# PJLab-ADG/DetZero

Measured on AMD Instinct MI355X. Metric: LiDAR frames/sec (160k pts, 0.1m voxels), higher is better.
Workload: dtype f32 as f16 pairs (hi+lo, 22-bit significand; 3 f16 MFMA per product, f32 accumulate)

## Files before the change

### detzero_amd/csrc/head_cand.hip

```cpp
#include "hgemm.h"

namespace dz {

constexpr int HC_C = 64;
constexpr int HC_CAND = 32;
constexpr int HC_THREADS = 192;
constexpr int HC_PIX_BYTES = HC_C * 4;
constexpr int HC_HROW = HC_PIX_BYTES + 16;
constexpr int HC_LDS_BYTES = 9 * HC_CAND * HC_HROW;
constexpr int HC_MAX_BRANCH = 4;

struct HcArgs {
    const unsigned char *shared;
    const unsigned long long *cand;
    const int *ncand;
    const unsigned char *w1, *w2;
    const float *s1, *b1, *s2, *b2;
    float *head;
    int h, w, k, cand_stride, w1_cout;
    int g_cout[HC_MAX_BRANCH], g_ooff[HC_MAX_BRANCH];
};

template <class M>
__global__ __launch_bounds__(HC_THREADS) __attribute__((amdgpu_waves_per_eu(2, 2))) void k_head_at_cand(HcArgs a) {
    extern __shared__ __attribute__((aligned(16))) unsigned char hid_s[];
    const int tid = threadIdx.x, lane = tid & 63, ty = tid >> 6;
    const int n = lane & 31, hh = lane >> 5;
    const int g = blockIdx.y, b = blockIdx.z;
    const int hw = a.h * a.w, hp = a.h + 2, wp = a.w + 2;
    const int ncand = min(min(a.ncand[b], a.k), a.cand_stride);
    const int slot = blockIdx.x * HC_CAND + n;
    if (blockIdx.x * HC_CAND >= ncand) return;
    const bool live = slot < ncand;
    int pix = 0, y = 0, x = 0;
    if (live) {
        const unsigned long long e = a.cand[(size_t)b * a.cand_stride + slot];
        const uint32_t flat = 0xFFFFFFFFu - (uint32_t)(e & 0xFFFFFFFFull);
        pix = (int)(flat % (uint32_t)hw);
        y = pix / a.w;
        x = pix - y * a.w;
    }
    const int hy = y + ty - 1;
    bool ok[3];
    const unsigned char *base[3];
#pragma unroll
    for (int tx = 0; tx < 3; ++tx) {
        const int hx = x + tx - 1;
        ok[tx] = live && hy >= 0 && hy < a.h && hx >= 0 && hx < a.w;
        base[tx] = a.shared + (ok[tx] ? (((size_t)b * hp + hy) * wp + hx) * HC_PIX_BYTES : (size_t)0);
    }
    f32x16 acc[2][3];
#pragma unroll
    for (int ct = 0; ct < 2; ++ct)
#pragma unroll
        for (int tx = 0; tx < 3; ++tx)
#pragma unroll
            for (int e = 0; e < 16; ++e) acc[ct][tx][e] = 0.f;
    const v4u zero4 = {0u, 0u, 0u, 0u};
    const unsigned char *const wrow = a.w1 + ((size_t)(g * HC_C + n) * HC_C) * 4;
    const size_t w_tap = (size_t)a.w1_cout * HC_C * 4, w_ct = (size_t)32 * HC_C * 4;
    for (int kc = 0; kc < HC_C / 32; ++kc) {
#pragma unroll
        for (int s = 0; s < 9; ++s) {
            const int ky = s / 3, kx = s - ky * 3;
            const size_t toff = (size_t)(ky * wp + kx) * HC_PIX_BYTES;
#pragma unroll
            for (int q = 0; q < 2; ++q) {
                const int koff = kc * 128 + q * 64 + hh * 32;
                v4u c_hi[2], c_lo[2], p_hi[3], p_lo[3];
#pragma unroll
                for (int ct = 0; ct < 2; ++ct) {
                    const unsigned char *wpn = wrow + s * w_tap + ct * w_ct + koff;
                    c_hi[ct] = *reinterpret_cast<const v4u *>(wpn);
                    c_lo[ct] = *reinterpret_cast<const v4u *>(wpn + 16);
                }
#pragma unroll
                for (int tx = 0; tx < 3; ++tx) {
                    p_hi[tx] = p_lo[tx] = zero4;
                    if (ok[tx]) {
                        const unsigned char *pp = base[tx] + toff + koff;
                        p_hi[tx] = *reinterpret_cast<const v4u *>(pp);
                        p_lo[tx] = *reinterpret_cast<const v4u *>(pp + 16);
                    }
                }
#pragma unroll
                for (int term = 3 - M::TERMS; term < 3; ++term)
#pragma unroll
                    for (int ct = 0; ct < 2; ++ct)
#pragma unroll
                        for (int tx = 0; tx < 3; ++tx)
                            acc[ct][tx] = M::mma(term == 0 ? c_lo[ct] : c_hi[ct], term == 1 ? p_lo[tx] : p_hi[tx], acc[ct][tx]);
            }
        }
    }
#pragma unroll
    for (int tx = 0; tx < 3; ++tx) {
        unsigned char *const row = hid_s + ((ty * 3 + tx) * HC_CAND + n) * HC_HROW;
#pragma unroll
        for (int ct = 0; ct < 2; ++ct) {
#pragma unroll
            for (int j = 0; j < 4; ++j) {
                const int ch = g * HC_C + ct * 32 + 8 * j + 4 * hh;
                float v[4];
#pragma unroll
                for (int e = 0; e < 4; ++e) v[e] = fmaxf(fmaf(acc[ct][tx][4 * j + e], a.s1[ch + e], a.b1[ch + e]), 0.f);
                uint2 hi, lo;
                split4<M>(v, hi, lo);
                if (!ok[tx]) hi = lo = make_uint2(0u, 0u);
                unsigned char *d = row + (ct * 4 + j) * 32 + hh * 8;
                *reinterpret_cast<uint2 *>(d) = hi;
                *reinterpret_cast<uint2 *>(d + 16) = lo;
            }
        }
    }
    __syncthreads();
    if (ty != 0) return;
    f32x16 out;
#pragma unroll
    for (int e = 0; e < 16; ++e) out[e] = 0.f;
    const unsigned char *const w2row = a.w2 + ((size_t)(g * 9 * 32 + n) * HC_C) * 4;
    for (int kc = 0; kc < HC_C / 32; ++kc) {
#pragma unroll
        for (int s = 0; s < 9; ++s) {
#pragma unroll
            for (int q = 0; q < 2; ++q) {
                const int koff = kc * 128 + q * 64 + hh * 32;
                const unsigned char *wpn = w2row + (size_t)s * 32 * HC_C * 4 + koff;
                const v4u c_hi = *reinterpret_cast<const v4u *>(wpn), c_lo = *reinterpret_cast<const v4u *>(wpn + 16);
                const unsigned char *pp = hid_s + (s * HC_CAND + n) * HC_HROW + koff;
                const v4u p_hi = *reinterpret_cast<const v4u *>(pp), p_lo = *reinterpret_cast<const v4u *>(pp + 16);
                if constexpr (M::TERMS == 3) {
                    out = M::mma(c_lo, p_hi, out);
                    out = M::mma(c_hi, p_lo, out);
                }
                out = M::mma(c_hi, p_hi, out);
            }
        }
    }
    if (live && hh == 0) {
        float *o = a.head + ((size_t)b * hw + pix) * 12 + a.g_ooff[g];
        const int gc = a.g_cout[g];
#pragma unroll
        for (int e = 0; e < 4; ++e) {
            if (e < gc) o[e] = fmaf(out[e], a.s2 ? a.s2[g * 32 + e] : 1.f, a.b2 ? a.b2[g * 32 + e] : 0.f);
        }
    }
}


constexpr int HF_CAND = 16;
constexpr int HF_HROW = HC_C + 4;

__global__ __launch_bounds__(HC_THREADS) void k_head_at_cand_f32(HcArgs a) {
    __shared__ __attribute__((aligned(16))) float hid_s[9 * HF_CAND * HF_HROW];
    __shared__ int pix_s[HF_CAND];
    __shared__ int ok_s[3][HF_CAND];
    const int tid = threadIdx.x, lane = tid & 63, ty = tid >> 6;
    const int r = lane & 15, g4 = lane >> 4;
    const int br = blockIdx.y, b = blockIdx.z;
    const int hw = a.h * a.w, hp = a.h + 2, wp = a.w + 2;
    const int ncand = min(min(a.ncand[b], a.k), a.cand_stride);
    if (blockIdx.x * HF_CAND >= ncand) return;
    const int slot = blockIdx.x * HF_CAND + r;
    const bool live = slot < ncand;
    int pix = 0, y = 0, x = 0;
    if (live) {
        const unsigned long long e = a.cand[(size_t)b * a.cand_stride + slot];
        const uint32_t flat = 0xFFFFFFFFu - (uint32_t)(e & 0xFFFFFFFFull);
        pix = (int)(flat % (uint32_t)hw);
        y = pix / a.w;
        x = pix - y * a.w;
    }
    const int hy = y + ty - 1;
    bool ok[3];
    const float *base[3];
    int okm = 0;
#pragma unroll
    for (int tx = 0; tx < 3; ++tx) {
        const int hx = x + tx - 1;
        ok[tx] = live && hy >= 0 && hy < a.h && hx >= 0 && hx < a.w;
        okm |= ok[tx] ? 1 << tx : 0;
        base[tx] = reinterpret_cast<const float *>(a.shared) + (ok[tx] ? (((size_t)b * hp + hy) * wp + hx) * HC_C : (size_t)0);
    }
    if (lane < HF_CAND) {
        ok_s[ty][lane] = okm;
        if (ty == 0) pix_s[lane] = live ? pix : -1;
    }
    __syncthreads();
    f32x4 acc[3][4];
#pragma unroll
    for (int tx = 0; tx < 3; ++tx)
#pragma unroll
        for (int nt = 0; nt < 4; ++nt) acc[tx][nt] = f32x4{0.f, 0.f, 0.f, 0.f};
    const float *const w1 = reinterpret_cast<const float *>(a.w1) + br * HC_C + r;
    for (int s = 0; s < 9; ++s) {
        const int ky = s / 3, kx = s - ky * 3;
        const size_t toff = (size_t)(ky * wp + kx) * HC_C;
#pragma unroll
        for (int kq = 0; kq < HC_C / 16; ++kq) {
            const int k0 = kq * 16 + g4 * 4;
            f32x4 av[3];
#pragma unroll
            for (int tx = 0; tx < 3; ++tx) {
                av[tx] = f32x4{0.f, 0.f, 0.f, 0.f};
                if (ok[tx]) av[tx] = *reinterpret_cast<const f32x4 *>(base[tx] + toff + k0);
            }
#pragma unroll
            for (int e = 0; e < 4; ++e) {
                float bv[4];
#pragma unroll
                for (int nt = 0; nt < 4; ++nt) bv[nt] = w1[((size_t)s * HC_C + k0 + e) * a.w1_cout + nt * 16];
#pragma unroll
                for (int tx = 0; tx < 3; ++tx)
#pragma unroll
                    for (int nt = 0; nt < 4; ++nt) acc[tx][nt] = __builtin_amdgcn_mfma_f32_16x16x4f32(av[tx][e], bv[nt], acc[tx][nt], 0, 0, 0);
            }
        }
    }
#pragma unroll
    for (int nt = 0; nt < 4; ++nt) {
        const int ch = br * HC_C + nt * 16 + r;
        const float sc = a.s1[ch], sh = a.b1[ch];
#pragma unroll
        for (int tx = 0; tx < 3; ++tx)
#pragma unroll
            for (int e = 0; e < 4; ++e) {
                const int c = 4 * g4 + e;
                const float v = fmaxf(fmaf(acc[tx][nt][e], sc, sh), 0.f);
                hid_s[((ty * 3 + tx) * HF_CAND + c) * HF_HROW + nt * 16 + r] = ((ok_s[ty][c] >> tx) & 1) ? v : 0.f;
            }
    }
    __syncthreads();
    if (ty != 0) return;
    f32x4 out = {0.f, 0.f, 0.f, 0.f};
    const float *const w2 = reinterpret_cast<const float *>(a.w2) + (size_t)br * 9 * HC_C * 16 + r;
    for (int s = 0; s < 9; ++s) {
#pragma unroll
        for (int kq = 0; kq < HC_C / 16; ++kq) {
            const int k0 = kq * 16 + g4 * 4;
            const f32x4 av = *reinterpret_cast<const f32x4 *>(hid_s + (s * HF_CAND + r) * HF_HROW + k0);
#pragma unroll
            for (int e = 0; e < 4; ++e) out = __builtin_amdgcn_mfma_f32_16x16x4f32(av[e], w2[((size_t)s * HC_C + k0 + e) * 16], out, 0, 0, 0);
        }
    }
    if (r < a.g_cout[br]) {
        const float sc = a.s2 ? a.s2[br * 16 + r] : 1.f, sh = a.b2 ? a.b2[br * 16 + r] : 0.f;
#pragma unroll
        for (int e = 0; e < 4; ++e) {
            const int px = pix_s[4 * g4 + e];
            if (px >= 0) a.head[((size_t)b * hw + px) * 12 + a.g_ooff[br] + r] = fmaf(out[e], sc, sh);
        }
    }
}

template <class M>
static int launch_head_at_cand(const HcArgs &a, int batch, int nbranch, hipStream_t stream) {
    static PerDeviceFlags lds_done;
    if (int rc_ = reserve_lds(reinterpret_cast<const void *>(&k_head_at_cand<M>), HC_LDS_BYTES, lds_done, "dz_head_at_candidates")) return rc_;
    hipLaunchKernelGGL((k_head_at_cand<M>), dim3(ceil_div(a.k, HC_CAND), nbranch, batch), dim3(HC_THREADS), HC_LDS_BYTES, stream, a);
    DZ_LAUNCH_CHECK();
    return DZ_OK;
}

}

using namespace dz;

extern "C" {

int dz_head_at_candidates_supported(int math, int channels) {
    return (math == DZ_MATH_F32 || math == DZ_MATH_F16X2 || math == DZ_MATH_BF16X2 || math == DZ_MATH_F16) && channels == HC_C ? 1 : 0;
}

int dz_head_at_candidates(const float *shared, int batch, int h, int w, const unsigned long long *cand, const int *d_ncand, int cand_stride,
                          int k, const float *w1, int w1_cout, const float *s1, const float *b1, const float *w2, const float *s2,
                          const float *b2, int nbranch, const int *h_g_cout, const int *h_g_ooff, float *head, int math, void *stream_) {
    hipStream_t stream = (hipStream_t)stream_;
    DZ_CHECK_ARG(dz_head_at_candidates_supported(math, HC_C), "dz_head_at_candidates: unknown math mode %d", math);
    DZ_CHECK_ARG(batch >= 0 && batch <= 65535 && h >= 1 && w >= 1 && k >= 1 && cand_stride >= k, "dz_head_at_candidates: bad sizes");
    DZ_CHECK_ARG(nbranch >= 1 && nbranch <= HC_MAX_BRANCH && w1_cout >= nbranch * HC_C && w1_cout % 32 == 0, "dz_head_at_candidates: bad branch layout");
    DZ_CHECK_ARG(shared && cand && d_ncand && w1 && s1 && b1 && w2 && head && h_g_cout && h_g_ooff, "dz_head_at_candidates: null pointer");
    if (batch == 0) return DZ_OK;
    HcArgs a{};
    for (int g = 0; g < nbranch; ++g) {
        DZ_CHECK_ARG(h_g_cout[g] >= 1 && h_g_cout[g] <= 4 && h_g_ooff[g] >= 0 && h_g_ooff[g] + h_g_cout[g] <= 12, "dz_head_at_candidates: bad columns of branch %d", g);
        a.g_cout[g] = h_g_cout[g];
        a.g_ooff[g] = h_g_ooff[g];
    }
    a.shared = reinterpret_cast<const unsigned char *>(shared);
    a.cand = cand; a.ncand = d_ncand;
    a.w1 = reinterpret_cast<const unsigned char *>(w1); a.w2 = reinterpret_cast<const unsigned char *>(w2);
    a.s1 = s1; a.b1 = b1; a.s2 = s2; a.b2 = b2; a.head = head;
    a.h = h; a.w = w; a.k = k; a.cand_stride = cand_stride; a.w1_cout = w1_cout;
    if (math == DZ_MATH_F32) {
        hipLaunchKernelGGL(k_head_at_cand_f32, dim3(ceil_div(k, HF_CAND), nbranch, batch), dim3(HC_THREADS), 0, stream, a);
        DZ_LAUNCH_CHECK();
        return DZ_OK;
    }
    if (math == DZ_MATH_F16X2) return launch_head_at_cand<MathF16>(a, batch, nbranch, stream);
    if (math == DZ_MATH_F16) return launch_head_at_cand<MathF16H>(a, batch, nbranch, stream);
    return launch_head_at_cand<MathBF16>(a, batch, nbranch, stream);
}

}
```

### detzero_amd/det_modules.py

```python
import contextlib
import os
from functools import partial

import numpy as np
import torch
import torch.nn as nn

from . import ops
from .lib import DetZeroHipError

PACKED_TABLES = bool(os.environ.get('DZ_TUNE_PACKED_TABLES'))

K3, S1, P1 = (3, 3, 3), (1, 1, 1), (1, 1, 1)


def _inference_only(module):
    if module.training:
        raise DetZeroHipError('%s: only the inference path is implemented on the HIP backend '
                              '(call .eval()); training is out of scope' % type(module).__name__)


def fold_bn(bn, conv_bias=None):
    w = bn.weight.detach().double()
    b = bn.bias.detach().double()
# ... 430 lines not shown
            e_prev, e = e, self._e('x_conv%d' % (i + 2))
            x = ops.spconv_forward(x, nbr_d, nxt, *self._p(dp, e_prev, e), None, True, in_level=level, math=mm)
            for bp in p[name]['blocks']:
                x = self._res_block(x, nbr, nxt, bp, e)
            nxt.act_exp = e
            out['x_conv%d' % (i + 2)] = (x, nxt)
            level = nxt
        dp = p['conv_out']
        nbr_d, _, nxt, ev = steps[4]
        ready(ev)
        e_prev, e = e, self._e('encoded')
        x = ops.spconv_forward(x, nbr_d, nxt, *self._p(dp, e_prev, e), None, True, in_level=level, math=mm)
        nxt.act_exp = e
        out['encoded'] = (x, nxt)
        return out

    def run(self, voxel_features, voxel_coords, batch_size, d_n=None, side_key=0, exact=False):
        return self.run_pyramid(self.build_pyramid(voxel_features, voxel_coords, batch_size, d_n, True, side_key, exact=exact))

    def _side_stream(self, dev, key=0):
        pool = self.__dict__.setdefault('_side_streams', {})
        k = (str(dev), key)
        if k not in pool:
            pool[k] = torch.cuda.Stream(device=dev, priority=int(os.environ.get('DZ_TUNE_SIDE_PRIORITY', '0')))
        return pool[k]

    def forward(self, batch_dict):
        _inference_only(self)
        vf = batch_dict['voxel_features'].float().contiguous()
        vc = batch_dict['voxel_coords'].int().contiguous()
        batch_size = batch_dict['batch_size']
        with torch.no_grad():
            res = self.run(vf, vc, batch_size, exact=True)

        def as_tensor(item):
            feats, level = item
            m = level.num_active()
            return SparseConvTensor(None, level.coords[:m], level.shape, batch_size, level=level, padded=(feats, level), math=self.math)
        batch_dict.update({'encoded_spconv_tensor': as_tensor(res['encoded']), 'encoded_spconv_tensor_stride': 8})
        batch_dict.update({'multi_scale_3d_features': {k: as_tensor(res[k]) for k in ('x_conv1', 'x_conv2', 'x_conv3', 'x_conv4')}})
        batch_dict.update({'multi_scale_3d_strides': {'x_conv1': 1, 'x_conv2': 2, 'x_conv3': 4, 'x_conv4': 8}})
        return batch_dict


class HeightCompression(nn.Module):

    def __init__(self, model_cfg, **kwargs):
        super().__init__()
        self.model_cfg = model_cfg
        self.num_bev_features = self.model_cfg.NUM_BEV_FEATURES

    def forward(self, batch_dict):
        t = batch_dict['encoded_spconv_tensor']
        feats, level = t._padded if t._padded is not None else (t.features, t._level)
        math = t._math if t._padded is not None else 0
        c = feats.shape[1]
        bev = ops.sparse_to_bev(feats, level, c, pad=1, math=math)
        e = int(getattr(level, 'act_exp', 0) or 0) if t._padded is not None else 0
        batch_dict['_nhwc_spatial_features'] = bev
        batch_dict['_nhwc_math'] = math
        batch_dict['_nhwc_exp'] = e
        plain = ops.pair16_to_f32(bev, math) if math else bev
        if e:
            plain = plain * (2.0 ** -e)
        batch_dict['spatial_features'] = plain[:, 1:-1, 1:-1, :].permute(0, 3, 1, 2)
        batch_dict['spatial_features_stride'] = batch_dict['encoded_spconv_tensor_stride']
        return batch_dict


def _conv_weight_taps(weight, cout_pad=None):
    co, ci, kh, kw = weight.shape
    w = weight.detach().permute(2, 3, 1, 0).reshape(kh * kw, ci, co).float()
    if cout_pad is not None and cout_pad > co:
        w = torch.cat([w, w.new_zeros(kh * kw, ci, cout_pad - co)], dim=2)
    return w.contiguous()


def _pad_vec(v, n, fill=0.0):
    if v.numel() == n:
        return v.contiguous()
    out = v.new_full((n,), fill)
    out[:v.numel()] = v
    return out


_WORKSPACE = [None]


@contextlib.contextmanager
def workspace(bufs):
    prev = _WORKSPACE[0]
    _WORKSPACE[0] = bufs
    try:
        yield
    finally:
        _WORKSPACE[0] = prev


def bordered_zeros(name, shape, dev):
    ws = _WORKSPACE[0]
    if ws is None:
        return torch.zeros(shape, dtype=torch.float32, device=dev)
    key = (name, tuple(shape), str(dev))
    buf = ws.get(key)
    if buf is None:
        buf = ws[key] = torch.zeros(shape, dtype=torch.float32, device=dev)
    return buf


def nchw_to_padded_nhwc(x, pad=1):
    b, c, h, w = x.shape
    out = x.new_zeros((b, h + 2 * pad, w + 2 * pad, c))
    out[:, pad:pad + h, pad:pad + w, :] = x.permute(0, 2, 3, 1)
    return out


def _recode(img, enc, math, e_src=0, e_dst=0):
    if ops.storage_math(enc) == ops.storage_math(math) and e_src == e_dst:
        return img
    plain = ops.pair16_to_f32(img, enc) if enc else img
    if e_src != e_dst:
        plain = plain * (2.0 ** (e_dst - e_src))
    return ops.pair16_from_f32(plain, math=math) if math else plain


SKIP_EMPTY_TILES = os.environ.get('DZ_TUNE_SKIP_EMPTY_TILES', '1') != '0'
SPARSE_BEV_INPUT = os.environ.get('DZ_TUNE_SPARSE_BEV', '1') != '0'
FIRST_BLOCK_WIDE_GROUPS = os.environ.get('DZ_TUNE_FIRST_BLOCK_WIDE', '1') != '0'
FUSED_DEBLOCK_PHASES = os.environ.get('DZ_TUNE_DEBLOCK_PHASES', '1') != '0'


def conv_layer(inp, in_shape, w, scale, shift, relu, out, out_shape, *, cin, in_cstride, in_coff=0, ksize=3,
               stride=1, in_off=0, out_cstride, out_coff=0, out_s=1, out_d=(0, 0), groups=1, cout_pad=None,
               g_cout=None, g_ooff=None, ho=None, wo=None, batch=1, math=0, out_f32=False, phase_groups=False, in_rowidx=None,
               in_row_channels=0, in_rows=0, in_tiles=None):
    if cout_pad is None:
        cout_pad = w.shape[-2] if math else w.shape[-1]
    ops.conv2d(dict(
        inp=inp.data_ptr(), out=out.data_ptr(), w=w.data_ptr(),
        scale=scale.data_ptr() if scale is not None else None,
        shift=shift.data_ptr() if shift is not None else None,
        batch=batch, ho=ho, wo=wo, in_hp=in_shape[0], in_wp=in_shape[1], in_cstride=in_cstride, in_coff=in_coff,
        cin=cin, kh=ksize, kw=ksize, stride=stride, in_off=in_off,
        out_hp=out_shape[0], out_wp=out_shape[1], out_cstride=out_cstride, out_coff=out_coff,
        out_sy=out_s, out_sx=out_s, out_dy=out_d[0], out_dx=out_d[1],
        groups=groups, cout_pad=cout_pad,
        g_cout=g_cout if g_cout is not None else [cout_pad], g_ooff=g_ooff if g_ooff is not None else [0],
        relu=1 if relu else 0, phase_groups=1 if phase_groups else 0,
        in_rowidx=in_rowidx.data_ptr() if in_rowidx is not None else None, in_row_channels=int(in_row_channels), in_rows=int(in_rows),
        in_tiles=in_tiles.data_ptr() if in_tiles is not None else None),
        math=math, out_f32=out_f32, tiles=in_tiles)


class BaseBEVBackbone(_Cached):

    def __init__(self, model_cfg, input_channels):
        super().__init__()
        self.model_cfg = model_cfg
        layer_nums = list(model_cfg.LAYER_NUMS)
        layer_strides = list(model_cfg.LAYER_STRIDES)
        num_filters = list(model_cfg.NUM_FILTERS)
        upsample_strides = list(model_cfg.UPSAMPLE_STRIDES)
        num_upsample_filters = list(model_cfg.NUM_UPSAMPLE_FILTERS)
        assert len(layer_nums) == len(layer_strides) == len(num_filters) == len(upsample_strides)
        c_in_list = [input_channels, *num_filters[:-1]]
        self.blocks = nn.ModuleList()
        self.deblocks = nn.ModuleList()
        for idx in range(len(layer_nums)):
            cur = [nn.ZeroPad2d(1),
                   nn.Conv2d(c_in_list[idx], num_filters[idx], kernel_size=3, stride=layer_strides[idx], padding=0, bias=False),
                   nn.BatchNorm2d(num_filters[idx], eps=1e-3, momentum=0.01), nn.ReLU()]
            for _ in range(layer_nums[idx]):
                cur.extend([nn.Conv2d(num_filters[idx], num_filters[idx], kernel_size=3, padding=1, bias=False),
                            nn.BatchNorm2d(num_filters[idx], eps=1e-3, momentum=0.01), nn.ReLU()])
            self.blocks.append(nn.Sequential(*cur))
            s = upsample_strides[idx]
            if not (isinstance(s, int) and s >= 1):
                raise DetZeroHipError('BaseBEVBackbone: only integer UPSAMPLE_STRIDES >= 1 are supported')
            self.deblocks.append(nn.Sequential(
                nn.ConvTranspose2d(num_filters[idx], num_upsample_filters[idx], s, stride=s, bias=False),
                nn.BatchNorm2d(num_upsample_filters[idx], eps=1e-3, momentum=0.01), nn.ReLU()))
        self.num_bev_features = sum(num_upsample_filters)
        self.layer_strides, self.upsample_strides = layer_strides, upsample_strides
        self.num_filters, self.num_upsample_filters = num_filters, num_upsample_filters
        self.input_channels = input_channels

    def plan(self):
        if self._plan is not None:
            return self._plan
        levels = []
        for idx, blk in enumerate(self.blocks):
            convs = []
            mods = list(blk)
            i = 1
            while i < len(mods):
                conv, bn = mods[i], mods[i + 1]
                scale, shift = fold_bn(bn, conv.bias)
                convs.append({'w': _conv_weight_taps(conv.weight), 'scale': scale, 'shift': shift,
                              'stride': conv.stride[0], 'cin': conv.in_channels, 'cout': conv.out_channels})
                if idx == 0 and len(convs) == 1 and conv.in_channels % 2 == 0:
                    wt_ = convs[0]['w']
                    c_half = conv.in_channels // 2
                    convs[0]['w_zmajor'] = wt_.view(wt_.shape[0], c_half, 2, wt_.shape[2]).permute(0, 2, 1, 3).reshape(wt_.shape).contiguous()
                i += 3
            de, dbn = self.deblocks[idx][0], self.deblocks[idx][1]
            scale, shift = fold_bn(dbn, de.bias)
            s = de.stride[0]
            wt = de.weight.detach().float()
            phases = [[{'w': wt[:, :, dy, dx].contiguous().unsqueeze(0).contiguous()} for dx in range(s)] for dy in range(s)]
            w_phases = wt.permute(2, 3, 0, 1).reshape(s * s, wt.shape[0], wt.shape[1]).contiguous()
            levels.append({'convs': convs, 'de': {'phases': phases, 'w_phases': w_phases, 'scale': scale, 'shift': shift, 's': s,
                                                  'cin': de.in_channels, 'cout': de.out_channels}})
        self._plan = levels
        return levels

    def sparse_input_ok(self, row_channels, slabs):
        cv = self.plan()[0]['convs'][0]
        return bool(self.math and SPARSE_BEV_INPUT and slabs == 2 and cv['stride'] == 1 and cv['cin'] == 2 * row_channels and
                    row_channels % 32 == 0 and cv['cout'] % 128 == 0)

    def _zero_response(self, lvl, h, w, rows_c, dev, nb0):
        e_in, e_mid = self._e('encoded'), self._e('spatial_features_2d')
        key = ('zero_resp', h, w, int(self.math), str(dev), int(nb0), e_in, e_mid)
        if key not in lvl:
            ridx = torch.full((nb0, h + 2, w + 2, 2), -1, dtype=torch.int32, device=dev)
            rows = torch.zeros((8, rows_c), dtype=torch.float32, device=dev)
            outs = []
            x, xh, xw, xc = None, h, w, 2 * rows_c
            with workspace(None):
                for ci, cv in enumerate(lvl['convs']):
                    if cv['stride'] != 1:
                        raise DetZeroHipError('BaseBEVBackbone: zero-response tiles need a stride-1 first block')
                    y = torch.zeros((nb0, xh + 2, xw + 2, cv['cout']), dtype=torch.float32, device=dev)
                    if ci == 0:
                        conv_layer(rows, (xh + 2, xw + 2), *self._p(cv, e_in, e_mid, key='w_zmajor'), True, y, (xh + 2, xw + 2), cin=cv['cin'],
                                   in_cstride=xc, ksize=3, stride=1, in_off=0, out_cstride=cv['cout'], out_d=(1, 1), ho=xh, wo=xw, batch=nb0,
                                   math=self.math, in_rowidx=ridx, in_row_channels=rows_c, in_rows=rows.shape[0])
                    else:
                        conv_layer(x, (xh + 2, xw + 2), *self._p(cv, e_mid, e_mid), True, y, (xh + 2, xw + 2), cin=cv['cin'], in_cstride=xc,
                                   ksize=3, stride=1, in_off=0, out_cstride=cv['cout'], out_d=(1, 1), ho=xh, wo=xw, batch=nb0, math=self.math)
                    outs.append(y[:1].clone())
                    x, xc = y, cv['cout']
            lvl[key] = outs
            order = lvl.setdefault('_zero_resp_keys', [])
            order.append(key)
            while len(order) > 4:
                lvl.pop(order.pop(0), None)
        return lvl[key]

    def _level_convs(self, li, lvl, x, xh, xw, xc, batch, dev, sparse_in=None, out_last=None):
        convs = lvl['convs']
        bufs = None
        tiles = zero = None
        e_in, e_mid = self._e('encoded'), self._e('spatial_features_2d')
        if sparse_in is not None and li == 0 and SKIP_EMPTY_TILES:
            nl = min(len(convs), 6) if all(cv['stride'] == 1 for cv in convs) else 1
            key = ('zero_resp', xh, xw, int(self.math), str(dev), int(batch), e_in, e_mid)
            if nl > 1 and key not in lvl and torch.cuda.is_current_stream_capturing():
                nl = 1
                if not getattr(self, '_warned_capture_nl1', False):
                    self._warned_capture_nl1 = True
                    import warnings
                    warnings.warn('BaseBEVBackbone: graph capture of a %d-frame pass without an eager pass of the same size before it - empty tiles '
                                  'are skipped at the first layer only (run one eager pass first to skip them in all six)' % batch)
            tiles = ops.bev_tile_list(sparse_in[1], xh, xw, nl)
            zero = self._zero_response(lvl, xh, xw, sparse_in[0].shape[1], dev, batch) if nl > 1 else None
        for ci, cv in enumerate(convs):
            s = cv['stride']
            oh, ow = (xh + 2 - 3) // s + 1, (xw + 2 - 3) // s + 1
            if bufs is None:
                bufs = [bordered_zeros('bev2d.l%d.%d' % (li, k), (batch, oh + 2, ow + 2, cv['cout']), dev) for k in range(2)]
            y = out_last if (out_last is not None and ci == len(convs) - 1) else bufs[ci % 2]
            if sparse_in is not None and li == 0 and ci == 0:
                rows, ridx = sparse_in
                wz, scz, shz = self._p(cv, e_in, e_mid, key='w_zmajor')
                conv_layer(rows, (xh + 2, xw + 2), wz, scz, shz, True, y, (oh + 2, ow + 2),
                           cin=cv['cin'], in_cstride=xc, ksize=3, stride=s, in_off=0, out_cstride=cv['cout'],
                           out_d=(1, 1), ho=oh, wo=ow, batch=batch, math=self.math, in_rowidx=ridx, in_row_channels=rows.shape[1],
                           in_rows=rows.shape[0], in_tiles=tiles[0] if tiles is not None else None)
                if tiles is not None:
                    ops.bev_fill_empty_tiles(tiles[0], batch, oh, ow, shz, True, cv['cout'], y, self.math)
            else:
                tl = tiles[ci] if (tiles is not None and ci < tiles.shape[0]) else None
                wc, scc, shc = self._p(cv, e_in if (li == 0 and ci == 0) else e_mid, e_mid)
                conv_layer(x, (xh + 2, xw + 2), wc, scc, shc, True, y, (oh + 2, ow + 2),
                           cin=cv['cin'], in_cstride=xc, ksize=3, stride=s, in_off=0, out_cstride=cv['cout'],
                           out_d=(1, 1), ho=oh, wo=ow, batch=batch, math=self.math, in_tiles=tl)
                if tl is not None:
                    ops.bev_fill_empty_tiles(tl, batch, oh, ow, shc, True, cv['cout'], y, self.math, zero_resp=zero[ci])
            x, xh, xw, xc = y, oh, ow, cv['cout']
        return x, xh, xw, xc

    def _level_deblock(self, lvl, x, xh, xw, xc, concat, coff, h, w, batch):
        de = lvl['de']
        s = de['s']
        ctot = self.num_bev_features
        e_mid = self._e('spatial_features_2d')
        if xh * s != h or xw * s != w:
            raise DetZeroHipError('BaseBEVBackbone: deblock output %dx%d does not match %dx%d' % (xh * s, xw * s, h, w))
        if self.math and 1 < s * s <= 8 and FUSED_DEBLOCK_PHASES:
            conv_layer(x, (xh + 2, xw + 2), *self._p(de, e_mid, e_mid, key='w_phases'), True, concat,
                       (h + 2, w + 2), cin=de['cin'], in_cstride=xc, ksize=1, stride=1, in_off=1,
                       out_cstride=ctot, out_coff=coff, out_s=s, out_d=(1, 1), ho=xh, wo=xw, batch=batch, math=self.math,
                       groups=s * s, g_cout=[de['cout']] * (s * s), g_ooff=[0] * (s * s), phase_groups=True)
            return coff + de['cout']
        for dy in range(s):
            for dx in range(s):
                conv_layer(x, (xh + 2, xw + 2), *self._p(de['phases'][dy][dx], e_mid, e_mid, scale=de['scale'], shift=de['shift']), True, concat,
                           (h + 2, w + 2), cin=de['cin'], in_cstride=xc, ksize=1, stride=1, in_off=1,
                           out_cstride=ctot, out_coff=coff, out_s=s, out_d=(dy + 1, dx + 1), ho=xh, wo=xw,
                           batch=batch, math=self.math)
        return coff + de['cout']

    def run(self, bev, batch, sparse_in=None):
        plan = self.plan()
        if sparse_in is not None:
            rows, ridx = sparse_in
            dev = rows.device
            h, w = ridx.shape[1] - 2, ridx.shape[2] - 2
        else:
            dev = bev.device
            h, w = bev.shape[1] - 2, bev.shape[2] - 2
        concat = bordered_zeros('bev2d.concat', (batch, h + 2, w + 2, self.num_bev_features), dev)
        x, xh, xw, xc = bev, h, w, (bev.shape[3] if sparse_in is None else 2 * rows.shape[1])
        coff = 0
        for li, lvl in enumerate(plan):
            x, xh, xw, xc = self._level_convs(li, lvl, x, xh, xw, xc, batch, dev, sparse_in=sparse_in if li == 0 else None)
            coff = self._level_deblock(lvl, x, xh, xw, xc, concat, coff, h, w, batch)
        return concat

    def grouped_fits(self, nb, h, w):
        plan = self.plan()
        xh, xw, worst = h, w, 0
        for lvl in plan:
            s = lvl['convs'][0]['stride']
            xh, xw = (xh + 2 - 3) // s + 1, (xw + 2 - 3) // s + 1
            worst = max(worst, (xh + 2) * (xw + 2) * lvl['convs'][-1]['cout'] * 4)
        return nb * worst < 2 ** 31

    def run_grouped(self, nb, group, consume, bev=None, sparse_in=None):
        plan = self.plan()
        if sparse_in is not None:
            rows, ridx = sparse_in
            dev = rows.device
            h, w = ridx.shape[1] - 2, ridx.shape[2] - 2
            cin0 = 2 * rows.shape[1]
        else:
            dev = bev.device
            h, w = bev.shape[1] - 2, bev.shape[2] - 2
            cin0 = bev.shape[3]
        l0 = plan[0]
        s0 = l0['convs'][0]['stride']
        h0, w0 = (h + 2 - 3) // s0 + 1, (w + 2 - 3) // s0 + 1
        c0 = l0['convs'][-1]['cout']
        if len(l0['convs']) < 2:
            raise DetZeroHipError('BaseBEVBackbone.run_grouped: the first block needs at least two convolutions')
        x0_all = bordered_zeros('bev2d.x0_all', (nb, h0 + 2, w0 + 2, c0), dev)
        widest = max([cin0] + [cv['cout'] for cv in l0['convs']])
        group1 = max(group, min(nb, (2 ** 31 - 1) // ((h + 2) * (w + 2) * widest * 4))) if FIRST_BLOCK_WIDE_GROUPS else group
        for g0 in range(0, nb, group1):
            ng = min(group1, nb - g0)
            sp = (rows, ridx[g0:g0 + ng]) if sparse_in is not None else None
            self._level_convs(0, l0, None if sp is not None else bev[g0:g0 + ng], h, w, cin0, ng, dev, sparse_in=sp, out_last=x0_all[g0:g0 + ng])
        outs = [(x0_all, h0, w0, c0)]
        x, xh, xw, xc = outs[0]
        for li in range(1, len(plan)):
            x, xh, xw, xc = self._level_convs(li, plan[li], x, xh, xw, xc, nb, dev)
            outs.append((x, xh, xw, xc))
        for g0 in range(0, nb, group):
            ng = min(group, nb - g0)
            concat = bordered_zeros('bev2d.concat', (ng, h + 2, w + 2, self.num_bev_features), dev)
            coff = 0
            for lvl, (x, xh, xw, xc) in zip(plan, outs):
                coff = self._level_deblock(lvl, x[g0:g0 + ng], xh, xw, xc, concat, coff, h, w, ng)
            consume(concat, g0, ng)

    def forward(self, data_dict):
        _inference_only(self)
        with torch.no_grad():
            bev = data_dict.get('_nhwc_spatial_features', None)
            enc = data_dict.get('_nhwc_math', 0)
            e_src = int(data_dict.get('_nhwc_exp', 0) or 0)
            if bev is None:
                bev, enc = nchw_to_padded_nhwc(data_dict['spatial_features'].float()), 0
                e_src = 0
            bev = _recode(bev, enc, self.math, e_src, self._e('encoded'))
            concat = self.run(bev, bev.shape[0])
        e_out = self._e('spatial_features_2d')
        data_dict['_nhwc_spatial_features_2d'] = concat
        data_dict['_nhwc_math'] = self.math
        data_dict['_nhwc_exp'] = e_out
        plain = ops.pair16_to_f32(concat, self.math) if self.math else concat
        if e_out:
            plain = plain * (2.0 ** -e_out)
        data_dict['spatial_features_2d'] = plain[:, 1:-1, 1:-1, :].permute(0, 3, 1, 2)
        return data_dict


class SeparateHead(nn.Module):

    def __init__(self, input_channels, sep_head_dict, init_bias=-2.19, use_bias=False):
# ... 288 lines not shown
```

Measured before the change: 1133.

## Stage candidate neighborhoods in LDS and pack two head branches per workgroup

The candidate-head kernel now first stages each candidate's 5x5 neighborhood of the shared feature map into LDS in two channel halves. The first 3x3 conv reads its inputs from LDS instead of issuing repeated global loads, and work is split across waves by output-channel tile. Two branches share one 768-thread workgroup, and both convolutions are software-pipelined with compile-time unrolled weight and activation prefetch and scheduling barriers. Separately, the zero-response cache in the backbone now pins entries created during graph capture so eviction cannot free buffers a captured graph still references, which is a correctness fix. The larger workgroup and LDS footprint may reduce occupancy, and the heavy unrolling may raise register pressure.

```diff
diff --git a/detzero_amd/csrc/head_cand.hip b/detzero_amd/csrc/head_cand.hip
--- a/detzero_amd/csrc/head_cand.hip
+++ b/detzero_amd/csrc/head_cand.hip
@@ -7,8 +7,17 @@
 constexpr int HC_THREADS = 192;
 constexpr int HC_PIX_BYTES = HC_C * 4;
 constexpr int HC_HROW = HC_PIX_BYTES + 16;
-constexpr int HC_LDS_BYTES = 9 * HC_CAND * HC_HROW;
+constexpr int HC_HID_BYTES = 9 * HC_CAND * HC_HROW;
 constexpr int HC_MAX_BRANCH = 4;
+constexpr int HC_BR = 2;
+constexpr int HC_WG = 64 * 6 * HC_BR;
+constexpr int HC_SROW = HC_PIX_BYTES / 2 + 16;
+constexpr int HC_STAGE_BYTES = 25 * HC_CAND * HC_SROW;
+constexpr int HC_ST = (25 * HC_CAND * 8 + HC_WG - 1) / HC_WG;
+constexpr int HC_LDS_BYTES = HC_BR * HC_HID_BYTES > HC_STAGE_BYTES ? HC_BR * HC_HID_BYTES : HC_STAGE_BYTES;
+constexpr int HC_IT = 2 * 9 * 2;
+static_assert(HC_WG % 256 == 0, "a thread stages one (candidate, 16-byte unit) of the pixels tid / 256 + i * HC_WG / 256");
+static_assert(HC_LDS_BYTES <= 160 * 1024, "LDS of a CU");
 
 struct HcArgs {
     const unsigned char *shared;
@@ -17,126 +26,193 @@
     const unsigned char *w1, *w2;
     const float *s1, *b1, *s2, *b2;
     float *head;
-    int h, w, k, cand_stride, w1_cout;
+    int h, w, k, cand_stride, w1_cout, nbranch;
     int g_cout[HC_MAX_BRANCH], g_ooff[HC_MAX_BRANCH];
 };
 
+template <int I, int N, class F>
+__device__ __forceinline__ void hc_for(F &&f) {
+    if constexpr (I < N) {
+        f(std::integral_constant<int, I>{});
+        hc_for<I + 1, N>(f);
+    }
+}
+
 template <class M>
-__global__ __launch_bounds__(HC_THREADS) __attribute__((amdgpu_waves_per_eu(2, 2))) void k_head_at_cand(HcArgs a) {
-    extern __shared__ __attribute__((aligned(16))) unsigned char hid_s[];
-    const int tid = threadIdx.x, lane = tid & 63, ty = tid >> 6;
+__global__ __launch_bounds__(HC_WG) void k_head_at_cand(HcArgs a) {
+    extern __shared__ __attribute__((aligned(16))) unsigned char lds[];
+    const int tid = threadIdx.x, lane = tid & 63, wv = __builtin_amdgcn_readfirstlane(tid >> 6);
+    const int brl = wv / 6, ty = (wv % 6) >> 1, ct = wv & 1;
     const int n = lane & 31, hh = lane >> 5;
-    const int g = blockIdx.y, b = blockIdx.z;
+    const int b = blockIdx.z;
+    const bool active = (int)blockIdx.y * HC_BR + brl < a.nbranch;
+    const int g = active ? blockIdx.y * HC_BR + brl : a.nbranch - 1;
     const int hw = a.h * a.w, hp = a.h + 2, wp = a.w + 2;
     const int ncand = min(min(a.ncand[b], a.k), a.cand_stride);
-    const int slot = blockIdx.x * HC_CAND + n;
     if (blockIdx.x * HC_CAND >= ncand) return;
-    const bool live = slot < ncand;
-    int pix = 0, y = 0, x = 0;
-    if (live) {
+    auto cell = [&](int c, int &pix, int &y, int &x) {
+        const int slot = blockIdx.x * HC_CAND + c;
+        pix = y = x = 0;
+        if (slot >= ncand) return false;
         const unsigned long long e = a.cand[(size_t)b * a.cand_stride + slot];
         const uint32_t flat = 0xFFFFFFFFu - (uint32_t)(e & 0xFFFFFFFFull);
         pix = (int)(flat % (uint32_t)hw);
         y = pix / a.w;
         x = pix - y * a.w;
-    }
+        return true;
+    };
+    const v4u zero4 = {0u, 0u, 0u, 0u};
+    const int sc = (tid >> 3) & 31, su = tid & 7, sj0 = tid >> 8;
+    int spix, sy, sx;
+    const bool slive = cell(sc, spix, sy, sx);
+    const unsigned char *const smap = a.shared + (size_t)b * hp * wp * HC_PIX_BYTES + su * 16;
+    unsigned char *const sdst = lds + sc * HC_SROW + su * 16;
+    v4u st[2][HC_ST];
+    unsigned int smask = 0;
+#pragma unroll
+    for (int i = 0; i < HC_ST; ++i) {
+        const int j = sj0 + i * (HC_WG / 256), dy = j / 5, dx = j - dy * 5;
+        const int py = sy + dy - 1, px = sx + dx - 1;
+        if (slive && j < 25 && py >= 0 && py < hp && px >= 0 && px < wp) smask |= 1u << i;
+    }
+    auto stage_load = [&](int kc) {
+#pragma unroll
+        for (int i = 0; i < HC_ST; ++i) {
+            const int j = sj0 + i * (HC_WG / 256), dy = j / 5, dx = j - dy * 5;
+            const size_t off = (smask >> i) & 1 ? ((size_t)(sy + dy - 1) * wp + (sx + dx - 1)) * HC_PIX_BYTES : (size_t)0;
+            st[kc][i] = *reinterpret_cast<const v4u *>(smap + off + kc * (HC_PIX_BYTES / 2));
+        }
+    };
+    auto stage_store = [&](int kc) {
+#pragma unroll
+        for (int i = 0; i < HC_ST; ++i) {
+            const int j = sj0 + i * (HC_WG / 256);
+            if (j < 25) *reinterpret_cast<v4u *>(sdst + j * HC_CAND * HC_SROW) = (smask >> i) & 1 ? st[kc][i] : zero4;
+        }
+    };
+    f32x16 acc[3];
+#pragma unroll
+    for (int tx = 0; tx < 3; ++tx)
+#pragma unroll
+        for (int e = 0; e < 16; ++e) acc[tx][e] = 0.f;
+    const unsigned char *const wbase = a.w1 + ((size_t)(g * HC_C + ct * 32) * HC_C) * 4;
+    const unsigned int wlane = n * HC_PIX_BYTES + hh * 32;
+    const size_t w_tap = (size_t)a.w1_cout * HC_C * 4;
+    const unsigned char *const prow = lds + (ty * 5 * HC_CAND + n) * HC_SROW + hh * 32;
+    v4u wq[2][2], pfh[2][3], pfl[3];
+    auto ldw = [&](auto it_t) {
+        constexpr int it = decltype(it_t)::value, kc = it / 18, s = (it % 18) / 2, q = it & 1;
+        const unsigned char *p = wbase + s * w_tap + kc * 128 + q * 64 + wlane;
+        wq[it & 1][0] = *reinterpret_cast<const v4u *>(p);
+        wq[it & 1][1] = *reinterpret_cast<const v4u *>(p + 16);
+    };
+    auto ldp = [&](auto it_t, auto lo_t) {
+        constexpr int it = decltype(it_t)::value, s = (it % 18) / 2, q = it & 1, ky = s / 3, kx = s - ky * 3;
+#pragma unroll
+        for (int tx = 0; tx < 3; ++tx) {
+            const unsigned char *p = prow + ((ky * 5 + tx + kx) * HC_CAND) * HC_SROW + q * 64;
+            if constexpr (decltype(lo_t)::value) pfl[tx] = *reinterpret_cast<const v4u *>(p + 16);
+            else pfh[it & 1][tx] = *reinterpret_cast<const v4u *>(p);
+        }
+    };
+    using lo_t = std::integral_constant<bool, true>;
+    using hi_t = std::integral_constant<bool, false>;
+    auto chunk = [&](auto kc_t) {
+        constexpr int kc = decltype(kc_t)::value;
+        ldp(std::integral_constant<int, kc * 18>{}, hi_t{});
+        hc_for<0, 18>([&](auto i_t) {
+            constexpr int i = decltype(i_t)::value, it = kc * 18 + i;
+            if constexpr (M::TERMS == 3) ldp(std::integral_constant<int, it>{}, lo_t{});
+            if constexpr (i + 1 < 18) ldp(std::integral_constant<int, it + 1>{}, hi_t{});
+            if constexpr (it + 1 < HC_IT) ldw(std::integral_constant<int, it + 1>{});
+            __builtin_amdgcn_sched_barrier(0);
+#pragma unroll
+            for (int term = 3 - M::TERMS; term < 3; ++term)
+#pragma unroll
+                for (int tx = 0; tx < 3; ++tx)
+                    acc[tx] = M::mma(term == 0 ? wq[it & 1][1] : wq[it & 1][0], term == 1 ? pfl[tx] : pfh[it & 1][tx], acc[tx]);
+            __builtin_amdgcn_sched_barrier(0);
+        });
+    };
+    ldw(std::integral_constant<int, 0>{});
+    stage_load(0);
+    stage_load(1);
+    stage_store(0);
+    __syncthreads();
+    chunk(std::integral_constant<int, 0>{});
+    __syncthreads();
+    stage_store(1);
+    __syncthreads();
+    chunk(std::integral_constant<int, 1>{});
+    int pix, y, x;
+    const bool live = cell(n, pix, y, x);
     const int hy = y + ty - 1;
     bool ok[3];
-    const unsigned char *base[3];
 #pragma unroll
     for (int tx = 0; tx < 3; ++tx) {
         const int hx = x + tx - 1;
         ok[tx] = live && hy >= 0 && hy < a.h && hx >= 0 && hx < a.w;
-        base[tx] = a.shared + (ok[tx] ? (((size_t)b * hp + hy) * wp + hx) * HC_PIX_BYTES : (size_t)0);
-    }
-    f32x16 acc[2][3];
-#pragma unroll
-    for (int ct = 0; ct < 2; ++ct)
-#pragma unroll
-        for (int tx = 0; tx < 3; ++tx)
-#pragma unroll
-            for (int e = 0; e < 16; ++e) acc[ct][tx][e] = 0.f;
-    const v4u zero4 = {0u, 0u, 0u, 0u};
-    const unsigned char *const wrow = a.w1 + ((size_t)(g * HC_C + n) * HC_C) * 4;
-    const size_t w_tap = (size_t)a.w1_cout * HC_C * 4, w_ct = (size_t)32 * HC_C * 4;
-    for (int kc = 0; kc < HC_C / 32; ++kc) {
-#pragma unroll
-        for (int s = 0; s < 9; ++s) {
-            const int ky = s / 3, kx = s - ky * 3;
-            const size_t toff = (size_t)(ky * wp + kx) * HC_PIX_BYTES;
-#pragma unroll
-            for (int q = 0; q < 2; ++q) {
-                const int koff = kc * 128 + q * 64 + hh * 32;
-                v4u c_hi[2], c_lo[2], p_hi[3], p_lo[3];
-#pragma unroll
-                for (int ct = 0; ct < 2; ++ct) {
-                    const unsigned char *wpn = wrow + s * w_tap + ct * w_ct + koff;
-                    c_hi[ct] = *reinterpret_cast<const v4u *>(wpn);
-                    c_lo[ct] = *reinterpret_cast<const v4u *>(wpn + 16);
-                }
-#pragma unroll
-                for (int tx = 0; tx < 3; ++tx) {
-                    p_hi[tx] = p_lo[tx] = zero4;
-                    if (ok[tx]) {
-                        const unsigned char *pp = base[tx] + toff + koff;
-                        p_hi[tx] = *reinterpret_cast<const v4u *>(pp);
-                        p_lo[tx] = *reinterpret_cast<const v4u *>(pp + 16);
-                    }
-                }
-#pragma unroll
-                for (int term = 3 - M::TERMS; term < 3; ++term)
-#pragma unroll
-                    for (int ct = 0; ct < 2; ++ct)
-#pragma unroll
-                        for (int tx = 0; tx < 3; ++tx)
-                            acc[ct][tx] = M::mma(term == 0 ? c_lo[ct] : c_hi[ct], term == 1 ? p_lo[tx] : p_hi[tx], acc[ct][tx]);
-            }
-        }
-    }
+    }
+    const bool outw = wv % 6 == 0 && active;
+    unsigned char *const hid_s = lds + brl * HC_HID_BYTES;
+    const unsigned char *const w2row = a.w2 + ((size_t)(g * 9 * 32 + n) * HC_C) * 4 + hh * 32;
+    v4u oq[5][2], op[2][2];
+    auto ldo = [&](auto it_t) {
+        constexpr int it = decltype(it_t)::value, kc = it / 18, s = (it % 18) / 2, q = it & 1;
+        const unsigned char *p = w2row + (size_t)s * 32 * HC_C * 4 + kc * 128 + q * 64;
+        oq[it % 5][0] = *reinterpret_cast<const v4u *>(p);
+        oq[it % 5][1] = *reinterpret_cast<const v4u *>(p + 16);
+    };
+    auto ldh = [&](auto it_t) {
+        constexpr int it = decltype(it_t)::value, kc = it / 18, s = (it % 18) / 2, q = it & 1;
+        const unsigned char *p = hid_s + (s * HC_CAND + n) * HC_HROW + kc * 128 + q * 64 + hh * 32;
+        op[it & 1][0] = *reinterpret_cast<const v4u *>(p);
+        op[it & 1][1] = *reinterpret_cast<const v4u *>(p + 16);
+    };
+    if (outw) hc_for<0, 4>(ldo);
+    float sc1[4][4], sh1[4][4];
+#pragma unroll
+    for (int j = 0; j < 4; ++j)
+#pragma unroll
+        for (int e = 0; e < 4; ++e) {
+            const int ch = g * HC_C + ct * 32 + 8 * j + 4 * hh + e;
+            sc1[j][e] = a.s1[ch];
+            sh1[j][e] = a.b1[ch];
+        }
+    __syncthreads();
 #pragma unroll
     for (int tx = 0; tx < 3; ++tx) {
         unsigned char *const row = hid_s + ((ty * 3 + tx) * HC_CAND + n) * HC_HROW;
 #pragma unroll
-        for (int ct = 0; ct < 2; ++ct) {
-#pragma unroll
-            for (int j = 0; j < 4; ++j) {
-                const int ch = g * HC_C + ct * 32 + 8 * j + 4 * hh;
-                float v[4];
-#pragma unroll
-                for (int e = 0; e < 4; ++e) v[e] = fmaxf(fmaf(acc[ct][tx][4 * j + e], a.s1[ch + e], a.b1[ch + e]), 0.f);
-                uint2 hi, lo;
-                split4<M>(v, hi, lo);
-                if (!ok[tx]) hi = lo = make_uint2(0u, 0u);
-                unsigned char *d = row + (ct * 4 + j) * 32 + hh * 8;
-                *reinterpret_cast<uint2 *>(d) = hi;
-                *reinterpret_cast<uint2 *>(d + 16) = lo;
-            }
-        }
-    }
-    __syncthreads();
-    if (ty != 0) return;
+        for (int j = 0; j < 4; ++j) {
+            float v[4];
+#pragma unroll
+            for (int e = 0; e < 4; ++e) v[e] = fmaxf(fmaf(acc[tx][4 * j + e], sc1[j][e], sh1[j][e]), 0.f);
+            uint2 hi, lo;
+            split4<M>(v, hi, lo);
+            if (!ok[tx]) hi = lo = make_uint2(0u, 0u);
+            unsigned char *d = row + (ct * 4 + j) * 32 + hh * 8;
+            *reinterpret_cast<uint2 *>(d) = hi;
+            *reinterpret_cast<uint2 *>(d + 16) = lo;
+        }
+    }
+    __syncthreads();
+    if (!outw) return;
     f32x16 out;
 #pragma unroll
     for (int e = 0; e < 16; ++e) out[e] = 0.f;
-    const unsigned char *const w2row = a.w2 + ((size_t)(g * 9 * 32 + n) * HC_C) * 4;
-    for (int kc = 0; kc < HC_C / 32; ++kc) {
-#pragma unroll
-        for (int s = 0; s < 9; ++s) {
-#pragma unroll
-            for (int q = 0; q < 2; ++q) {
-                const int koff = kc * 128 + q * 64 + hh * 32;
-                const unsigned char *wpn = w2row + (size_t)s * 32 * HC_C * 4 + koff;
-                const v4u c_hi = *reinterpret_cast<const v4u *>(wpn), c_lo = *reinterpret_cast<const v4u *>(wpn + 16);
-                const unsigned char *pp = hid_s + (s * HC_CAND + n) * HC_HROW + koff;
-                const v4u p_hi = *reinterpret_cast<const v4u *>(pp), p_lo = *reinterpret_cast<const v4u *>(pp + 16);
-                if constexpr (M::TERMS == 3) {
-                    out = M::mma(c_lo, p_hi, out);
-                    out = M::mma(c_hi, p_lo, out);
-                }
-                out = M::mma(c_hi, p_hi, out);
-            }
-        }
-    }
+    ldh(std::integral_constant<int, 0>{});
+    hc_for<0, HC_IT>([&](auto it_t) {
+        constexpr int it = decltype(it_t)::value;
+        if constexpr (it + 1 < HC_IT) ldh(std::integral_constant<int, it + 1>{});
+        if constexpr (it + 4 < HC_IT) ldo(std::integral_constant<int, it + 4>{});
+        if constexpr (M::TERMS == 3) {
+            out = M::mma(oq[it % 5][1], op[it & 1][0], out);
+            out = M::mma(oq[it % 5][0], op[it & 1][1], out);
+        }
+        out = M::mma(oq[it % 5][0], op[it & 1][0], out);
+        __builtin_amdgcn_sched_barrier(0);
+    });
     if (live && hh == 0) {
         float *o = a.head + ((size_t)b * hw + pix) * 12 + a.g_ooff[g];
         const int gc = a.g_cout[g];
@@ -257,7 +333,7 @@
 static int launch_head_at_cand(const HcArgs &a, int batch, int nbranch, hipStream_t stream) {
     static PerDeviceFlags lds_done;
     if (int rc_ = reserve_lds(reinterpret_cast<const void *>(&k_head_at_cand<M>), HC_LDS_BYTES, lds_done, "dz_head_at_candidates")) return rc_;
-    hipLaunchKernelGGL((k_head_at_cand<M>), dim3(ceil_div(a.k, HC_CAND), nbranch, batch), dim3(HC_THREADS), HC_LDS_BYTES, stream, a);
+    hipLaunchKernelGGL((k_head_at_cand<M>), dim3(ceil_div(a.k, HC_CAND), ceil_div(nbranch, HC_BR), batch), dim3(HC_WG), HC_LDS_BYTES, stream, a);
     DZ_LAUNCH_CHECK();
     return DZ_OK;
 }
@@ -291,7 +367,7 @@
     a.cand = cand; a.ncand = d_ncand;
     a.w1 = reinterpret_cast<const unsigned char *>(w1); a.w2 = reinterpret_cast<const unsigned char *>(w2);
     a.s1 = s1; a.b1 = b1; a.s2 = s2; a.b2 = b2; a.head = head;
-    a.h = h; a.w = w; a.k = k; a.cand_stride = cand_stride; a.w1_cout = w1_cout;
+    a.h = h; a.w = w; a.k = k; a.cand_stride = cand_stride; a.w1_cout = w1_cout; a.nbranch = nbranch;
     if (math == DZ_MATH_F32) {
         hipLaunchKernelGGL(k_head_at_cand_f32, dim3(ceil_div(k, HF_CAND), nbranch, batch), dim3(HC_THREADS), 0, stream, a);
         DZ_LAUNCH_CHECK();
diff --git a/detzero_amd/det_modules.py b/detzero_amd/det_modules.py
--- a/detzero_amd/det_modules.py
+++ b/detzero_amd/det_modules.py
@@ -606,6 +606,21 @@
         math=math, out_f32=out_f32, tiles=in_tiles)
 
 
+def _zero_resp_handout(lvl, key, capturing, keep=4):
+    order = lvl.setdefault('_zero_resp_keys', [])
+    pinned = lvl.setdefault('_zero_resp_pinned', set())
+    if key in order:
+        order.remove(key)
+    order.append(key)
+    if capturing:
+        pinned.add(key)
+    loose = [k for k in order if k not in pinned]
+    for k in loose[:max(0, len(loose) - keep)]:
+        order.remove(k)
+        lvl.pop(k, None)
+    return lvl[key]
+
+
 class BaseBEVBackbone(_Cached):
 
     def __init__(self, model_cfg, input_channels):
@@ -696,11 +711,7 @@
                     outs.append(y[:1].clone())
                     x, xc = y, cv['cout']
             lvl[key] = outs
-            order = lvl.setdefault('_zero_resp_keys', [])
-            order.append(key)
-            while len(order) > 4:
-                lvl.pop(order.pop(0), None)
-        return lvl[key]
+        return _zero_resp_handout(lvl, key, torch.cuda.is_current_stream_capturing())
 
     def _level_convs(self, li, lvl, x, xh, xw, xc, batch, dev, sparse_in=None, out_last=None):
         convs = lvl['convs']
```

After: 1136, median of 6. No clear change (+0.3%).
